# HENDRIX-ZT2/pyaudiorestoration

Hardware: AMD Instinct MI355X
Metric: Msamples/sec resampled (192 kHz varispeed) (higher is better)
Workload: dtype f32 near taps, far taps (|n| >= 3) as float16 hi + lo x 2^-12 filter banks on v_mfma_f32_16x16x32_f16 with f32 accumulation / f64 positions

## Files before the change

pyaudiorestoration_amd/csrc/sinc2.hip:

```cpp
#define PAR_WANT_BANK2 1
#include "par_common.h"
#include "pos_plan.h"
#include "sinc_taps_gen.h"
#include "sinc_common.h"
#define PAR_COLD_FN __forceinline__
#include "sinc_block.h"
#ifndef PAR_COLD_FN_GIVEN
#error "sinc_block.h was included before PAR_COLD_FN was defined: the cold functions would stay out of line"
#endif
#include <algorithm>
#include <atomic>
#include <limits.h>
#include <type_traits>

constexpr int kMaxTilesPerWave = 23;
#ifndef PAR_S2_EXP
#define PAR_S2_EXP 0
#endif

namespace par {

typedef _Float16 half8v __attribute__((ext_vector_type(8)));
typedef _Float16 half2v __attribute__((ext_vector_type(2)));
typedef float float4v __attribute__((ext_vector_type(4)));
// ... 32 lines not shown
  int64_t n_big;
  int64_t n_full;
  int64_t n_tiles;
  int n_edge;
  int64_t out_stride;
  FusedArgs fa;
  const float4* tab;
  TapModes tmd;
};
constexpr int kEdgeWaveOut = 128;
constexpr int kEdgeWavesPerTile = kSincTileOutputs / kEdgeWaveOut;
constexpr int kTileEdge = 0x100;

__device__ __forceinline__ float sinpi_poly(float z) {
  float p = -0.00737043094f;
  p = fmaf(p, z, 0.0821458866f);
  p = fmaf(p, z, -0.599264529f);
  p = fmaf(p, z, 2.55016404f);
  p = fmaf(p, z, -5.16771278f);
  return fmaf(p, z, 3.14159265f);
}

__device__ __forceinline__ _Float16 hi16(float x) { return (_Float16)(fabsf(x) < 6.103515625e-05f ? 0.0f : x); }
#define S2_HI(x) hi16(x)

__device__ __forceinline__ unsigned pack_h2(float a, float b) {
  const half2v h = {(_Float16)a, (_Float16)b};
  return __builtin_bit_cast(unsigned, h);
}
__device__ __forceinline__ float h_lo(unsigned w) { return (float)__builtin_bit_cast(half2v, w)[0]; }
__device__ __forceinline__ float h_hi(unsigned w) { return (float)__builtin_bit_cast(half2v, w)[1]; }


__device__ __forceinline__ void dma_dword(const float* gptr, const void* lds) {
  const unsigned la = (unsigned)(uintptr_t)(const __attribute__((address_space(3))) void*)lds;
  asm volatile("s_mov_b32 m0, %1\n\tglobal_load_lds_dword %0, off" ::"v"(gptr), "s"(__builtin_amdgcn_readfirstlane(la)) : "memory", "m0");
}
__device__ __forceinline__ void dma_dwordx4(const void* gptr, const void* lds) {
  const unsigned la = (unsigned)(uintptr_t)(const __attribute__((address_space(3))) void*)lds;
  asm volatile("s_mov_b32 m0, %1\n\tglobal_load_lds_dwordx4 %0, off" ::"v"(gptr), "s"(__builtin_amdgcn_readfirstlane(la)) : "memory", "m0");
}

__device__ __forceinline__ void dma_chunk128(const float* base, unsigned lane_bytes, const void* lds) {
  const unsigned la = (unsigned)(uintptr_t)(const __attribute__((address_space(3))) void*)lds;
  const unsigned long long b = (unsigned long long)(uintptr_t)base;
  const unsigned long long bs = ((unsigned long long)(unsigned)__builtin_amdgcn_readfirstlane((int)(b >> 32)) << 32) |
                                (unsigned)__builtin_amdgcn_readfirstlane((int)(unsigned)b);
  asm volatile("s_mov_b32 m0, %2\n\tglobal_load_lds_dword %0, %1\n\tglobal_load_lds_dword %0, %1 offset:256"
               ::"v"(lane_bytes), "s"(bs), "s"(__builtin_amdgcn_readfirstlane(la)) : "memory", "m0");
}

__device__ __forceinline__ void dma_chunk256(const float* base, unsigned lane_bytes, const void* lds) {
  const unsigned la = (unsigned)(uintptr_t)(const __attribute__((address_space(3))) void*)lds;
  const unsigned long long b = (unsigned long long)(uintptr_t)base;
  const unsigned long long bs = ((unsigned long long)(unsigned)__builtin_amdgcn_readfirstlane((int)(b >> 32)) << 32) |
                                (unsigned)__builtin_amdgcn_readfirstlane((int)(unsigned)b);
  asm volatile("s_mov_b32 m0, %2\n\tglobal_load_lds_dword %0, %1\n\tglobal_load_lds_dword %0, %1 offset:256\n\t"
               "global_load_lds_dword %0, %1 offset:512\n\tglobal_load_lds_dword %0, %1 offset:768"
               ::"v"(lane_bytes), "s"(bs), "s"(__builtin_amdgcn_readfirstlane(la)) : "memory", "m0");
}

__device__ __forceinline__ void wave_lds_fence() {
  __builtin_amdgcn_fence(__ATOMIC_RELEASE, "wavefront");
  __builtin_amdgcn_wave_barrier();
  __builtin_amdgcn_fence(__ATOMIC_ACQUIRE, "wavefront");
}

__device__ __forceinline__ int clamp64(int n) { return n < 0 ? 0 : (n > 64 ? 64 : n); }
__device__ __forceinline__ unsigned long long prefix(int n) { return n >= 64 ? ~0ull : ((1ull << n) - 1ull); }

struct S2Row {
  int c;
  float s, ep;
  bool bad;
};
template <bool SECOND = true>
__device__ __forceinline__ S2Row s2_place_row(const uint4 ra, const uint4 rb, const int u, const int cbase, const float uf,
                                              const float u2f, const float tw1, const float tw0, const float tolf) {
  const unsigned m = ra.x;
  const bool second = SECOND && (unsigned)u > (m & 31u);
  const float F = __uint_as_float(second ? rb.y : ra.y), e1 = __uint_as_float(second ? rb.z : ra.z),
              e2 = __uint_as_float(second ? rb.w : ra.w);
  const int irel = (int)(second ? rb.x : ra.x) >> 16;
  const bool last = (unsigned)u == ((m >> kRecLastShift) & 63u);
  const float frac = fmaf(u2f, e2, fmaf(uf, e1, F));
  const float e = fmaf(e2, last ? tw0 : tw1, e1);
  const float ri = rintf(frac);
// ... 170 lines not shown
    const float G = 3.14159265f * g, w = G * sr, w2m = w * w, G32 = 32.0f * G;
    float re, im;
    if constexpr (MODE == 3) {
      re = m6 * (1.98412698e-4f * kMs);
      im = 0.0f;
    } else {
      re = m5 * (1.38888889e-3f * kMs);
      im = m5 * (w * -(1.19047619e-3f * kMs));
    }
#define S3_MOM_STEP(Mi, A0, A1, B0)                                   \
    {                                                                 \
      const float al_ = (A1) != 0.0f ? fmaf(w2m, -((A1) * kMs), (A0) * kMs) : (A0) * kMs, be_ = w * -((B0) * kMs);       \
      const float nre_ = fmaf(-G32, im, (Mi) * al_), nim_ = fmaf(G32, re, (Mi) * be_); \
      re = nre_;                                                      \
      im = nim_;                                                      \
    }
    if constexpr (MODE == 3) S3_MOM_STEP(m5, 1.38888889e-3f, 0.0f, 1.19047619e-3f)
    S3_MOM_STEP(m4, 8.33333333e-3f, 0.0f, 6.94444444e-3f)
    S3_MOM_STEP(m3, 4.16666667e-2f, 0.0f, 3.33333333e-2f)
    S3_MOM_STEP(M0[2], 1.66666667e-1f, 5.0e-2f, 1.25e-1f)
    S3_MOM_STEP(M0[1], 0.5f, 0.125f, 3.33333333e-1f)
    S3_MOM_STEP(M0[0], 1.0f, 1.66666667e-1f, 0.5f)
#undef S3_MOM_STEP
    const float S = sr * spq, C = __builtin_amdgcn_cosf(0.5f * sr);
    return fmaf(-g, fmaf(C, re, -(S * im)), unity);
    }
  }
}
template <int MODE, int NCH = 1, class LDS>
__device__ __forceinline__ float s3_out_row(const LDS& L, const int ci, const float sr, const float epr, const int wsK, const int ch = 0) {
  return s3_out_math<MODE>(s3_out_load<MODE, NCH>(L, ci, wsK, ch), sr, epr);
}

template <class LDS>
__device__ __forceinline__ float2 s3_convert_load(const LDS& L, const int chunk, const int l) {
  const int ix = (chunk * kPass + 2 * l) & (kRingF - 1);
  return *reinterpret_cast<const float2*>(&L.ring[ix]);
}
template <class LDS>
__device__ __forceinline__ bool s3_convert_math(LDS& L, const int chunk, const int l, const float2 xx) {
  const int wi = chunk * kPass + 2 * l;
  const int ix = wi & (kRingF - 1), ih = wi & (kRingH - 1);
  const float x0 = xx.x, x1 = xx.y;
  const float am = fmaxf(fabsf(x0), fabsf(x1));
  const bool ok = !(__ballot(!(fabsf(x0) < kImgMax) || !(fabsf(x1) < kImgMax)) != 0ull ||
                    (__ballot(am >= kQuiet) == 0ull && __ballot(am > 0.0f) != 0ull));
  if ((chunk & 7) == 0 && l < 2) *reinterpret_cast<float2*>(&L.ring_tail[ix]) = xx;
  if ((chunk & 7) == 7 && l == kWave - 1) *reinterpret_cast<float2*>(&L.ring_head[2]) = xx;
  const float s0 = x0 * kImgScale, s1 = x1 * kImgScale;
  const half2v h = {S2_HI(s0), S2_HI(s1)};
  const half2v lo = {(_Float16)((s0 - (float)h[0]) * 4096.0f), (_Float16)((s1 - (float)h[1]) * 4096.0f)};
  *reinterpret_cast<half2v*>(&L.img[0][ih]) = h;
  *reinterpret_cast<half2v*>(&L.img[1][ih]) = lo;
  return ok;
}
template <class LDS>
__device__ __forceinline__ bool s3_convert(LDS& L, const int chunk, const int l) {
  return s3_convert_math(L, chunk, l, s3_convert_load(L, chunk, l));
}

template <class LDS>
__device__ __forceinline__ bool s3_convert_ch(LDS& L, const int chunk, const int l, const int ch, const bool mirrors) {
  const int wi = chunk * kPass + 2 * l;
  const int ix = wi & (kRingF - 1), ih = wi & (kRingH - 1);
  const float4v xx = *reinterpret_cast<const float4v*>(&L.ring[2 * ix]);
  const float x0 = ch ? xx[1] : xx[0], x1 = ch ? xx[3] : xx[2];
  const float am = fmaxf(fabsf(x0), fabsf(x1));
  const bool ok = !(__ballot(!(fabsf(x0) < kImgMax) || !(fabsf(x1) < kImgMax)) != 0ull ||
                    (__ballot(am >= kQuiet) == 0ull && __ballot(am > 0.0f) != 0ull));
  if (mirrors) {
    if ((chunk & 7) == 0 && l < 2) *reinterpret_cast<float4v*>(&L.ring_tail[2 * ix]) = xx;
    if ((chunk & 7) == 7 && l == kWave - 1) *reinterpret_cast<float4v*>(&L.ring_head[4]) = xx;
  }
  const float s0 = x0 * kImgScale, s1 = x1 * kImgScale;
  const half2v h = {S2_HI(s0), S2_HI(s1)};
  const half2v lo = {(_Float16)((s0 - (float)h[0]) * 4096.0f), (_Float16)((s1 - (float)h[1]) * 4096.0f)};
  *reinterpret_cast<half2v*>(&L.img[2 * ch][ih]) = h;
  *reinterpret_cast<half2v*>(&L.img[2 * ch + 1][ih]) = lo;
  return ok;
}

constexpr float kEpMaxMom = 0.0125f / (1.0f - 0.0125f);
constexpr float kEpMom5 = 0.0105f / (1.0f - 0.0105f), kEpMom5Lo = 0.95f * kEpMom5;
#ifndef PAR_S3_SHARE_OUT
#define PAR_S3_SHARE_OUT 1
#endif
#ifndef PAR_S3_PIN_MONO
#define PAR_S3_PIN_MONO 0
#endif
template <int NCH, int KIND>
__device__ __forceinline__ void sinc_pipe_body(const S2Args& a, const int bx, S3Lds<NCH, KIND != 1>& L) {
  static_assert(NCH == 1 || NCH == 2, "mono, or an interleaved stereo file");
  static_assert(KIND == 0 || KIND == 3 || NCH == 1, "the stereo form takes every stream");
  static_assert(KIND != 3 || NCH == 2, "one channel of FRAMES");
  constexpr bool kPick = KIND == 3;
  constexpr bool kTwo = NCH == 2 && !kPick;
  constexpr bool kMom = KIND != 1;
  constexpr bool kEarly = NCH == 1 && KIND == 2;
  const int l = threadIdx.x & (kWave - 1);
  if (bx < a.n_edge) {
    if constexpr (KIND == 1) return;
    else {
    const int e = bx / kEdgeWavesPerTile, w = bx % kEdgeWavesPerTile;
    const int64_t T = e == 0 ? 0 : a.n_full - 3 + e;
    const int64_t jw = T * kSincTileOutputs + (int64_t)w * kEdgeWaveOut;
    const int nrem = (int)(a.len_out - jw < (int64_t)kEdgeWaveOut ? (a.len_out - jw > 0 ? a.len_out - jw : 0) : kEdgeWaveOut);
    float* const piece = reinterpret_cast<float*>(&L);
    static_assert(sizeof(L) >= fused_capw(2 * NCH, NCH) * NCH * sizeof(float), "the wave's span fits the stream's LDS");
    if constexpr (kPick) {
      static_assert(sizeof(L) >= fused_capw(2, 1) * sizeof(float), "the wave's span fits the stream's LDS");
      if (nrem > 0)
        fused_wave<1, 32, 2, false>(a.len_out, a.sig, nullptr, 2, a.len_in, 32, a.tab, a.tmd, a.out, nullptr, a.out_stride, a.fa, piece, l,
// ... 27 lines not shown
    if (a.n_edge > 0 && (Ta + l == 0 || Ta + l >= a.n_full - 2)) hd_fl |= 1 | kTileEdge;
    hd_dA = (int)d;
    if constexpr (KIND == 1 || KIND == 2) {
      const bool any_slow = __ballot(l < my_tiles && Ta + l < Tb && (h.flags & kTileMaySlow) != 0) != 0ull;
      if (any_slow != (KIND == 2)) return;
    }
  }
  half8v fr[kBank2Frags];
  {
    const uint4* src = reinterpret_cast<const uint4*>(kBank2Frags32) + l;
#pragma unroll
    for (int f = 0; f < kBank2Frags; ++f) fr[f] = __builtin_bit_cast(half8v, src[f * kWave]);
  }
  half8v fmr[kBank3Frags];
  if constexpr (kMom) {
    const uint4* src = reinterpret_cast<const uint4*>(kBank3Frags32) + l;
#pragma unroll
    for (int f = 0; f < kBank3Frags; ++f) fmr[f] = __builtin_bit_cast(half8v, src[f * kWave]);
  }
  {
    uint4* z = reinterpret_cast<uint4*>(&L.img[0][0]);
    const uint4 zero = {0u, 0u, 0u, 0u};
#pragma unroll
    for (int i = 0; i < (int)(sizeof(L.img) / 16 / kWave); ++i) z[i * kWave + l] = zero;
  }
  const float tolf = (float)((fabs((double)A0) + 2.0e7) * 1.2e-16 + 2.0e-10) + 2.0e-7f;
  const int nJ = (int)(Jb - Ja);
  float* const outW = a.out + (kPick ? a.out_stride : (int64_t)NCH) * Ja;
  const uint4* const recW = reinterpret_cast<const uint4*>(a.rec) + (Ja >> kRecShift);
  const uint4* const rec2W = reinterpret_cast<const uint4*>(a.rec2) + (Ja >> kRecShift);
  const int blk_max = (int)(((a.len_out + kRec - 1) >> kRecShift) - (Ja >> kRecShift)) - 1;

  int j0 = 0;
  int wbase = 0, conv_next = 0, conv_lo = 0, dma_next = 0, dma_bad = INT_MAX, mode = 0, pk = 0;
  int regime = 1;
  int rbA = 0, rbB = 0, rbC = 0;

  const uint4* const rec_lane = (l < 8 ? recW : rec2W) + (l & 7);
  auto fetch_records = [&](int buf, int blk0) {
    if (l < 16) dma_dwordx4(rec_lane + (blk0 < 0 ? 0 : blk0), &L.recs[buf][0]);
  };
  int dma_klo = 0, dma_khi = -1;
  const float* ring_src = a.sig;
  auto ring_restart = [&]() {
    const long long o = A0 + wbase;
    ring_src = a.sig + NCH * o;
    const long long klo = o >= 0 ? 0 : (-o + kPass - 1) / kPass, khi = ((long long)a.len_in - (kPick ? 1 : 0) - o) / kPass - 1;
    dma_klo = (int)(klo > 0x3fffffff ? 0x3fffffff : klo);
    dma_khi = (int)(khi > 0x3fffffff ? 0x3fffffff : (khi < -1 ? -1 : khi));
  };
  const unsigned lane_bytes = 4u * (unsigned)l;
  auto chunk_dma = [&](int k) {
    const bool inside = k >= dma_klo && k <= dma_khi;
    if (!inside) dma_bad = k < dma_bad ? k : dma_bad;
    const float* src = inside ? ring_src + (long long)(kPass * NCH) * k : a.sig;
    if constexpr (NCH == 2) dma_chunk256(src, lane_bytes, &L.ring[(k & 7) * (kPass * 2)]);
    else dma_chunk128(src, lane_bytes, &L.ring[(k & 7) * kPass]);
  };
  auto push_tile = [&](int64_t T) {
    if (l == 0) {
      const int slot = atomicAdd(a.redo_count, 1);
      a.redo_list[slot] = (int)T;
    }
  };
  if (stream_id == 0 && a.n_full < a.n_tiles && a.n_edge == 0) push_tile(a.n_full);

  struct Placed {
    S2Row R[2];
    int nt[2];
    int fl0, fl1, tend;
    int epm;
  };
  int tc_T = -1, tc_dA0 = 0, tc_dA1 = 0, tc_fl0 = 0, tc_fl1 = 0;
  struct PlaceRecs {
    uint4 ra0, rb0, ra1, rb1;
  };
  auto place_load = [&](int j, int buf, int rb) {
    const int t5 = (j & (kRec - 1)) + l;
    const int bi = ((j >> kRecShift) - rb + (t5 >> kRecShift)) & 7;
    const uint4* rp = &L.recs[buf][0];
    return PlaceRecs{rp[bi], rp[8 + bi], rp[(bi + 2) & 7], rp[8 + ((bi + 2) & 7)]};
  };
  auto place_impl = [&](int j, int buf, int rb, auto early, const PlaceRecs& RR) {
    Placed P;
    const int T = j >> 10;
    P.tend = (T + 1) << 10;
    if (T != tc_T) {
      tc_T = T;
      tc_dA0 = __builtin_amdgcn_readlane(hd_dA, T);
      tc_dA1 = __builtin_amdgcn_readlane(hd_dA, T + 1);
      tc_fl0 = __builtin_amdgcn_readlane(hd_fl, T);
      tc_fl1 = __builtin_amdgcn_readlane(hd_fl, T + 1);
    }
    const int dA0 = tc_dA0, dA1 = tc_dA1;
    P.fl0 = tc_fl0;
    P.fl1 = tc_fl1;
    const int t5 = (j & (kRec - 1)) + l;
    const int u = t5 & (kRec - 1);
    uint4 ra0, rb0, ra1, rb1;
    if constexpr (decltype(early)::value) {
      ra0 = RR.ra0, rb0 = RR.rb0, ra1 = RR.ra1, rb1 = RR.rb1;
    } else {
      const int bi = ((j >> kRecShift) - rb + (t5 >> kRecShift)) & 7;
      const uint4* rp = &L.recs[buf][0];
      ra0 = rp[bi], rb0 = rp[8 + bi], ra1 = rp[(bi + 2) & 7], rb1 = rp[8 + ((bi + 2) & 7)];
    }
    const int uc = u - kRec / 2;
    const float uf = (float)uc, u2f = uf * uf, tw1 = fmaf(2.0f, uf, 1.0f), tw0 = tw1 - 2.0f;
    P.nt[0] = clamp64(P.tend - j);
    P.nt[1] = clamp64(P.tend - j - 64);
    if (__ballot((unsigned)u > (ra0.x & 31u) || (unsigned)u > (ra1.x & 31u)) == 0ull) {
      P.R[0] = s2_place_row<false>(ra0, rb0, u, (l < P.nt[0] ? dA0 : dA1) + uc, uf, u2f, tw1, tw0, tolf);
      P.R[1] = s2_place_row<false>(ra1, rb1, u, (l < P.nt[1] ? dA0 : dA1) + uc, uf, u2f, tw1, tw0, tolf);
    } else {
      P.R[0] = s2_place_row(ra0, rb0, u, (l < P.nt[0] ? dA0 : dA1) + uc, uf, u2f, tw1, tw0, tolf);
      P.R[1] = s2_place_row(ra1, rb1, u, (l < P.nt[1] ? dA0 : dA1) + uc, uf, u2f, tw1, tw0, tolf);
    }
    P.epm = max(__float_as_int(P.R[0].ep), __float_as_int(P.R[1].ep));
    return P;
  };
  auto place = [&](int j, int buf, int rb) { return place_impl(j, buf, rb, std::false_type{}, PlaceRecs{}); };

  S3Pass P;
  P.nok[0] = P.nok[1] = 0;
  P.j = P.ws = 0;
  P.c[0] = P.c[1] = 0;
  P.s[0] = P.s[1] = P.ep[0] = P.ep[1] = 0.0f;

  auto out_pass = [&](auto mode_tag, const S3Pass& Q, float (&res)[2], const int ch = 0) {
    constexpr int MODE = decltype(mode_tag)::value;
    const int wsK = Q.ws - wbase;
#pragma unroll
    for (int r = 0; r < 2; ++r) {
      int ci = Q.c[r] - Q.ws;
      ci = ci < 0 ? 0 : (ci > kPass - 1 ? kPass - 1 : ci);
      float sr = Q.s[r], epr = Q.ep[r];
#if !PAR_S3_SHARE_OUT
      if (NCH == 2 && ch == 1) asm volatile("" : "+v"(sr), "+v"(epr));
#endif
      res[r] = s3_out_row<MODE, NCH>(L, ci, sr, epr, wsK, ch);
    }
  };
  auto store_pass = [&](const S3Pass& Q, const float (&res)[2]) {
#pragma unroll
    for (int r = 0; r < 2; ++r)
      if (l < Q.nok[r] && !(PAR_S2_EXP & 4)) {
        if constexpr (kPick) outW[(int64_t)((unsigned)Q.j + 64u * r + (unsigned)l) * a.out_stride] = res[r];
        else outW[(unsigned)Q.j + 64u * r + (unsigned)l] = res[r];
      }
  };
  auto store_pass2 = [&](const S3Pass& Q, const float (&res0)[2], const float (&res1)[2]) {
#pragma unroll
    for (int r = 0; r < 2; ++r)
      if (l < Q.nok[r] && !(PAR_S2_EXP & 4))
        reinterpret_cast<float2*>(outW)[(unsigned)Q.j + 64u * r + (unsigned)l] = make_float2(res0[r], res1[r]);
  };
  auto convert_chunk = [&](int chunk) -> bool {
    if constexpr (kPick) {
      return s3_convert_ch(L, chunk, l, 0, true);
    } else if constexpr (NCH == 2) {
      const bool ok0 = s3_convert_ch(L, chunk, l, 0, true);
      const bool ok1 = s3_convert_ch(L, chunk, l, 1, false);
      return ok0 && ok1;
    } else {
      return s3_convert(L, chunk, l);
    }
  };

#if PAR_S2_EXP & 128
#define S3_COUNT(k) do { if (l == 0) atomicAdd(a.redo_count + (k), 1); } while (0)
#else
#define S3_COUNT(k) do { } while (0)
#endif
  auto start_run = [&]() -> bool {
    for (;;) {
      if (j0 >= nJ) return false;
      S3_COUNT(1);
      __builtin_amdgcn_s_waitcnt(0x0F70);
      wave_lds_fence();
      const int buf = pk & 3;
      fetch_records(buf, j0 >> kRecShift);
      __builtin_amdgcn_s_waitcnt(0x0F70);
      wave_lds_fence();
      const Placed Q = place(j0, buf, j0 >> kRecShift);
      const int tend = Q.tend;
      int nv[2] = {clamp64(nJ - j0), clamp64(nJ - j0 - 64)};
      const unsigned long long b0 = __ballot(Q.R[0].bad || !(Q.R[0].ep <= kEpMaxMom)) & prefix(nv[0]),
                               b1 = __ballot(Q.R[1].bad || !(Q.R[1].ep <= kEpMaxMom)) & prefix(nv[1]);
      const unsigned long long bad_here = (b0 & prefix(Q.nt[0])) | (b1 & prefix(Q.nt[1]));
      const bool bad_next = ((b0 & ~prefix(Q.nt[0])) | (b1 & ~prefix(Q.nt[1])) | (unsigned long long)((Q.fl1 & 1) && tend < nJ)) != 0ull;
      if (bad_next) {
        nv[0] = nv[0] < Q.nt[0] ? nv[0] : Q.nt[0];
        nv[1] = nv[1] < Q.nt[1] ? nv[1] : Q.nt[1];
      }
      bool skip = (Q.fl0 & 1) || bad_here != 0ull;
      const unsigned long long gen = (__ballot(1.0f + Q.R[0].ep != 1.0f) & prefix(nv[0])) | (__ballot(1.0f + Q.R[1].ep != 1.0f) & prefix(nv[1]));
      const int ws = __builtin_amdgcn_readfirstlane(Q.R[0].c) & ~7;
      S3Pass N;
#pragma unroll
      for (int r = 0; r < 2; ++r) {
        N.c[r] = Q.R[r].c;
        N.s[r] = Q.R[r].s;
        N.ep[r] = Q.R[r].ep;
        const unsigned long long in = __ballot(Q.R[r].c - ws < kPass);
        N.nok[r] = __popcll(in & prefix(nv[r]));
      }
      N.j = j0;
      N.ws = ws;
      const unsigned long long steep = (__ballot(Q.R[0].ep > kEpMom5) & prefix(nv[0])) | (__ballot(Q.R[1].ep > kEpMom5) & prefix(nv[1]));
      const int want = gen == 0ull ? 1 : (steep == 0ull ? 2 : 3);
      if (!kMom && want != 1) skip = true;
      if (!skip) {
        bool rebuild = mode != 1;
        const int lo_need = ws - 39 - wbase;
        if (mode == 0 || lo_need < kPass * (dma_next - 8) + kPass || lo_need < 0 || lo_need > kPass * dma_next || ws - wbase > (1 << 20)) {
          __builtin_amdgcn_s_waitcnt(0x0F70);
          wbase = ws - 39;
          dma_next = 0;
          dma_bad = INT_MAX;
          rebuild = true;
          ring_restart();
        }
        const int wsK = ws - wbase;
        regime = want;
        if (rebuild) {
          mode = 1;
          conv_lo = conv_next = (wsK - 39) >> 7;
        }
        const int conv_target = want == 1 ? (wsK + 300 + 127) >> 7 : (wsK + 465) >> 7;
        const int need_lo = (wsK - 39) >> 7;
        if (conv_next < need_lo) conv_lo = conv_next = need_lo;
        int conv_end = conv_target > conv_next ? conv_target : conv_next;
        if (need_lo < conv_lo || need_lo < conv_end - 4) {
          conv_lo = conv_next = need_lo;
          conv_end = conv_target > need_lo ? conv_target : need_lo;
        }
        while (dma_next < conv_end + 2) chunk_dma(dma_next++);
        const int jn = j0 + N.nok[0] + N.nok[1];
        rbA = jn >> kRecShift;
        rbB = (jn + 120) >> kRecShift;
        fetch_records((pk + 1) & 3, rbA);
        fetch_records((pk + 2) & 3, rbB);
        __builtin_amdgcn_s_waitcnt(0x0F70);
        wave_lds_fence();
        if (!skip) {
#pragma unroll 1
          while (conv_next < conv_end) {
            if (conv_next >= dma_bad) {
              skip = true;
              break;
            }
            const bool ok = convert_chunk(conv_next);
            if (!ok) {
              skip = true;
              break;
            }
            ++conv_next;
          }
        }
        if (!skip && conv_next + 1 >= dma_bad) skip = true;
      }
      if (skip) {
        if (!(Q.fl0 & kTileEdge)) push_tile(Ta + (j0 >> 10));
        j0 = tend;
        mode = 0;
        continue;
      }
      wave_lds_fence();
      const int offs = ws - wbase - 31;
      if (kMom && regime == 3) bank_image3m<kMom, true>(L, fr, fmr, offs, l);
      else if (kMom && regime == 2) bank_image3m<kMom, false>(L, fr, fmr, offs, l);
      else bank_image3m<false>(L, fr, fmr, offs, l);
      wave_lds_fence();
      j0 += N.nok[0] + N.nok[1];
      ++pk;
      rbC = (j0 + 240) >> kRecShift;
      const bool full = N.nok[1] >= 1 && N.nok[0] + N.nok[1] >= 120;
      if (full) {
        P = N;
        return true;
      }
      float res[2];
      if (kMom && regime == 3) out_pass(std::integral_constant<int, kMom ? 3 : 1>{}, N, res);
      else if (kMom && regime == 2) out_pass(std::integral_constant<int, kMom ? 2 : 1>{}, N, res);
      else out_pass(std::integral_constant<int, 1>{}, N, res);
      if constexpr (kTwo) {
        float res1[2];
        wave_lds_fence();
        if (regime == 3) bank_image3m<true, true>(L, fr, fmr, offs, l, 1);
        else if (regime == 2) bank_image3m<true, false>(L, fr, fmr, offs, l, 1);
        else bank_image3m<false>(L, fr, fmr, offs, l, 1);
        wave_lds_fence();
        if (regime == 3) out_pass(std::integral_constant<int, 3>{}, N, res1, 1);
        else if (regime == 2) out_pass(std::integral_constant<int, 2>{}, N, res1, 1);
        else out_pass(std::integral_constant<int, 1>{}, N, res1, 1);
        store_pass2(N, res, res1);
      } else {
        store_pass(N, res);
      }
    }
  };

#if PAR_S2_EXP & 64
  unsigned long long s3t_[4] = {0, 0, 0, 0}, s3last_ = __builtin_readcyclecounter();
  const unsigned long long s3start_ = s3last_;
#endif
  auto hot = [&](auto mode_tag) {
    constexpr int MODE = decltype(mode_tag)::value;
    j0 = __builtin_amdgcn_readfirstlane(j0);
    wbase = __builtin_amdgcn_readfirstlane(wbase);
    conv_next = __builtin_amdgcn_readfirstlane(conv_next);
    dma_next = __builtin_amdgcn_readfirstlane(dma_next);
    dma_bad = __builtin_amdgcn_readfirstlane(dma_bad);
    pk = __builtin_amdgcn_readfirstlane(pk);
    rbA = __builtin_amdgcn_readfirstlane(rbA);
    rbB = __builtin_amdgcn_readfirstlane(rbB);
    rbC = __builtin_amdgcn_readfirstlane(rbC);
    for (;;) {
#if PAR_S2_EXP & 64
      const unsigned long long tA_ = __builtin_readcyclecounter();
#endif
      if constexpr (NCH == 2) asm volatile("s_waitcnt vmcnt(7)" ::: "memory");
      else asm volatile("s_waitcnt vmcnt(5)" ::: "memory");
#if PAR_S2_EXP & 64
      const unsigned long long tB_ = __builtin_readcyclecounter();
      s3t_[0] += tB_ - tA_;
      s3t_[1] += tA_ - s3last_;
      s3last_ = tB_;
      s3t_[2] += 1;
#endif
      wave_lds_fence();
      S3Pass N;
      bool ok;
      int wsK;
      auto place_next = [&](auto early, const PlaceRecs& RR) {
      const Placed Q = place_impl(j0, pk & 3, rbA, early, RR);
      const unsigned long long bad = __ballot(Q.R[0].bad || Q.R[1].bad || Q.epm > __float_as_int(kEpMaxMom));
      const unsigned long long gen = __ballot(Q.epm > 0x33800000);
      bool tier = true;
      if constexpr (MODE == 2) tier = __ballot(Q.epm > __float_as_int(kEpMom5)) == 0ull;
      if constexpr (MODE == 3) tier = __ballot(Q.epm > __float_as_int(kEpMom5Lo)) != 0ull;
      const int ws = __builtin_amdgcn_readfirstlane(Q.R[0].c) & ~7;
#pragma unroll
      for (int r = 0; r < 2; ++r) {
        N.c[r] = Q.R[r].c;
        N.s[r] = Q.R[r].s;
        N.ep[r] = Q.R[r].ep;
        N.nok[r] = __popcll(__ballot(Q.R[r].c - ws < kPass));
      }
      N.j = j0;
      N.ws = ws;
      wsK = ws - wbase;
      const int d = kPass * conv_next - wsK;
      ok = (((Q.fl0 | Q.fl1) & 1) == 0) & (bad == 0ull) & (j0 + kPass <= nJ) & (N.nok[0] + N.nok[1] >= 120) &
           (MODE == 1 ? gen == 0ull : gen != 0ull) & tier & ((unsigned)(d - 161) <= 312u) & (conv_next + 1 < dma_bad) &
           ((unsigned)((j0 >> kRecShift) - rbA) <= 1u);
      };
      float res[2];
      bool cok;
      if constexpr (kEarly) {
        const PlaceRecs RR = place_load(j0, pk & 3, rbA);
        const float2 cxx = s3_convert_load(L, conv_next, l);
        S3Gather G[2];
        const int wsP = P.ws - wbase;
#pragma unroll
        for (int r = 0; r < 2; ++r) {
          int ci = P.c[r] - P.ws;
          ci = ci < 0 ? 0 : (ci > kPass - 1 ? kPass - 1 : ci);
          G[r] = s3_out_load<MODE, NCH>(L, ci, wsP);
        }
        __builtin_amdgcn_sched_barrier(0);
        place_next(std::true_type{}, RR);
        const S3Frags X = bank_load(L, wsK - 31, l);
        __builtin_amdgcn_sched_barrier(0);
        if constexpr (MODE == 2) {
          res[0] = s3_out_math<MODE>(G[0], P.s[0], P.ep[0]);
          asm volatile("" : "+v"(res[0]));
          asm volatile("" ::"v"(G[0].Mh[3]));
          __builtin_amdgcn_sched_barrier(0);
          res[1] = s3_out_math<MODE>(G[1], P.s[1], P.ep[1]);
          bank_math<true, false>(L, fr, fmr, X, l);
          asm volatile("" : "+v"(res[1]));
          asm volatile("" ::"v"(G[1].Mh[3]));
#pragma unroll
          for (int i = 0; i < 28; ++i) {
            __builtin_amdgcn_sched_group_barrier(0x008, 1, 0);
            __builtin_amdgcn_sched_group_barrier(0x002, 2, 0);
          }
        } else {
#pragma unroll
          for (int r = 0; r < 2; ++r) res[r] = s3_out_math<MODE>(G[r], P.s[r], P.ep[r]);
          asm volatile("" : "+v"(res[0]), "+v"(res[1]));
          __builtin_amdgcn_sched_barrier(0);
          bank_math<MODE != 1, MODE == 3>(L, fr, fmr, X, l);
        }
        int oki = __builtin_amdgcn_readfirstlane((int)ok);
        asm volatile("" : "+s"(oki));
        ok = oki != 0;
        cok = s3_convert_math(L, conv_next, l, cxx);
        fetch_records((pk + 2) & 3, rbC);
        chunk_dma(dma_next);
        store_pass(P, res);
      } else {
      if constexpr (!kTwo) place_next(std::false_type{}, PlaceRecs{});
      out_pass(mode_tag, P, res);
      if constexpr (kTwo) {
        float res1[2];
        asm volatile("" : "+v"(res[0]), "+v"(res[1]));
        bank_image3m<MODE != 1, MODE == 3>(L, fr, fmr, P.ws - wbase - 31, l, 1);
        out_pass(mode_tag, P, res1, 1);
        asm volatile("" : "+v"(res1[0]), "+v"(res1[1]));
        place_next(std::false_type{}, PlaceRecs{});
        const int offs = wsK - 31;
        bank_image3m<MODE != 1, MODE == 3>(L, fr, fmr, offs, l, 0);
        const bool c0 = s3_convert_ch(L, conv_next, l, 0, true);
        const bool c1 = s3_convert_ch(L, conv_next - 1, l, 1, false);
        cok = c0 && c1;
        fetch_records((pk + 2) & 3, rbC);
        chunk_dma(dma_next);
        store_pass2(P, res, res1);
      } else {
        const int offs = wsK - 31;
#if PAR_S3_PIN_MONO
        asm volatile("" : "+v"(res[0]), "+v"(res[1]));
#endif
        bank_image3m<MODE != 1, MODE == 3>(L, fr, fmr, offs, l);
        cok = convert_chunk(conv_next);
        fetch_records((pk + 2) & 3, rbC);
        chunk_dma(dma_next);
        store_pass(P, res);
      }
      }
      wave_lds_fence();
      ++conv_next;
      ++dma_next;
      if (!cok) mode = 0;
      S3_COUNT(2);
#if PAR_S2_EXP & 128
      if (!(ok && cok)) {
        if (((Q.fl0 | Q.fl1) & 1) != 0 || bad != 0ull) S3_COUNT(3);
        else if (!(j0 + kPass <= nJ)) S3_COUNT(4);
        else if (!(N.nok[1] >= 1 && N.nok[0] + N.nok[1] >= 120)) S3_COUNT(5);
        else if (!(MODE == 1 ? gen == 0ull : gen != 0ull)) S3_COUNT(6);
        else if (!(d >= 161 && d <= 473)) S3_COUNT(7);
        else if (!(conv_next < dma_bad)) S3_COUNT(9);
        else if (!((unsigned)((j0 >> kRecShift) - rbA) <= 1u)) S3_COUNT(11);
        else if (!cok) S3_COUNT(10);
        else S3_COUNT(8);
      }
#endif
      if (!(ok && cok)) {
        if constexpr (kTwo)
          if (mode != 0 && !s3_convert_ch(L, conv_next - 1, l, 1, false)) mode = 0;
        return;
      }
      P = N;
      j0 += N.nok[0] + N.nok[1];
      ++pk;
      rbA = rbB;
      rbB = rbC;
      rbC = (j0 + 240) >> kRecShift;
    }
  };

  while (start_run()) {
    if (kMom && regime == 3) hot(std::integral_constant<int, kMom ? 3 : 1>{});
    else if (kMom && regime == 2) hot(std::integral_constant<int, kMom ? 2 : 1>{});
    else hot(std::integral_constant<int, 1>{});
  }
  __builtin_amdgcn_s_waitcnt(0x0F70);
#if PAR_S2_EXP & 64
  if (l == 0) {
    unsigned long long* o = g_s2_phase + (size_t)stream_id * 16;
    o[0] = s3t_[0];
    o[1] = s3t_[1];
    o[2] = s3t_[2];
    o[3] = __builtin_readcyclecounter() - s3start_;
    o[6] = s3t_[2];
  }
#endif
}

template <int NCH, int KIND>
__global__ __launch_bounds__(kWave, KIND == 1 ? 3 : 2) void k_sinc_pipe(const S2Args a) {
  __shared__ S3Lds<NCH, KIND != 1> L;
  sinc_pipe_body<NCH, KIND>(a, (int)blockIdx.x, L);
}

constexpr int kBatchFiles = kFusedBatchMax;
struct S2Batch {
  int n;
  int first[kBatchFiles + 1];
  S2Args f[kBatchFiles];
};
static_assert(sizeof(S2Batch) <= 3584, "kernel arguments fit the 4 KB segment");
// ... 105 lines not shown
```

Before: 175,000.

## Strength-reduce hot-loop bookkeeping and fold exit checks into one integer margin

```diff
diff --git a/pyaudiorestoration_amd/csrc/sinc2.hip b/pyaudiorestoration_amd/csrc/sinc2.hip
--- a/pyaudiorestoration_amd/csrc/sinc2.hip
+++ b/pyaudiorestoration_amd/csrc/sinc2.hip
@@ -88,27 +88,24 @@
 __device__ __forceinline__ float h_hi(unsigned w) { return (float)__builtin_bit_cast(half2v, w)[1]; }
 
 
-__device__ __forceinline__ void dma_dword(const float* gptr, const void* lds) {
-  const unsigned la = (unsigned)(uintptr_t)(const __attribute__((address_space(3))) void*)lds;
+__device__ __forceinline__ unsigned lds_addr(const void* lds) {
+  return (unsigned)(uintptr_t)(const __attribute__((address_space(3))) void*)lds;
+}
+__device__ __forceinline__ void dma_dword(const float* gptr, const unsigned la) {
   asm volatile("s_mov_b32 m0, %1\n\tglobal_load_lds_dword %0, off" ::"v"(gptr), "s"(__builtin_amdgcn_readfirstlane(la)) : "memory", "m0");
 }
-__device__ __forceinline__ void dma_dwordx4(const void* gptr, const void* lds) {
-  const unsigned la = (unsigned)(uintptr_t)(const __attribute__((address_space(3))) void*)lds;
+__device__ __forceinline__ void dma_dwordx4(const void* gptr, const unsigned la) {
   asm volatile("s_mov_b32 m0, %1\n\tglobal_load_lds_dwordx4 %0, off" ::"v"(gptr), "s"(__builtin_amdgcn_readfirstlane(la)) : "memory", "m0");
 }
 
-__device__ __forceinline__ void dma_chunk128(const float* base, unsigned lane_bytes, const void* lds) {
-  const unsigned la = (unsigned)(uintptr_t)(const __attribute__((address_space(3))) void*)lds;
-  const unsigned long long b = (unsigned long long)(uintptr_t)base;
+__device__ __forceinline__ void dma_chunk128(const unsigned long long b, unsigned lane_bytes, const unsigned la) {
   const unsigned long long bs = ((unsigned long long)(unsigned)__builtin_amdgcn_readfirstlane((int)(b >> 32)) << 32) |
                                 (unsigned)__builtin_amdgcn_readfirstlane((int)(unsigned)b);
   asm volatile("s_mov_b32 m0, %2\n\tglobal_load_lds_dword %0, %1\n\tglobal_load_lds_dword %0, %1 offset:256"
                ::"v"(lane_bytes), "s"(bs), "s"(__builtin_amdgcn_readfirstlane(la)) : "memory", "m0");
 }
 
-__device__ __forceinline__ void dma_chunk256(const float* base, unsigned lane_bytes, const void* lds) {
-  const unsigned la = (unsigned)(uintptr_t)(const __attribute__((address_space(3))) void*)lds;
-  const unsigned long long b = (unsigned long long)(uintptr_t)base;
+__device__ __forceinline__ void dma_chunk256(const unsigned long long b, unsigned lane_bytes, const unsigned la) {
   const unsigned long long bs = ((unsigned long long)(unsigned)__builtin_amdgcn_readfirstlane((int)(b >> 32)) << 32) |
                                 (unsigned)__builtin_amdgcn_readfirstlane((int)(unsigned)b);
   asm volatile("s_mov_b32 m0, %2\n\tglobal_load_lds_dword %0, %1\n\tglobal_load_lds_dword %0, %1 offset:256\n\t"
@@ -345,52 +342,62 @@
   return s3_out_math<MODE>(s3_out_load<MODE, NCH>(L, ci, wsK, ch), sr, epr);
 }
 
+__device__ __forceinline__ unsigned long long s3_convert_verdict(const float x0, const float x1) {
+  const float am = fmaxf(fabsf(x0), fabsf(x1));
+  const unsigned long long big = __ballot(!(fabsf(x0) < kImgMax) || !(fabsf(x1) < kImgMax));
+  const unsigned long long loud = __ballot(am >= kQuiet), some = __ballot(am > 0.0f);
+  return big | (loud == 0ull ? some : 0ull);
+}
+template <int NCH, class LDS, class V>
+__device__ __forceinline__ void s3_ring_mirrors(LDS& L, const int w0, const int l, const int ix, const V xx) {
+  const int slot = w0 & (7 * kPass);
+  if (slot == 0) {
+    __builtin_amdgcn_wave_barrier();
+    if (l < 2) *reinterpret_cast<V*>(&L.ring_tail[NCH * ix]) = xx;
+  }
+  if (slot == 7 * kPass) {
+    __builtin_amdgcn_wave_barrier();
+    if (l == kWave - 1) *reinterpret_cast<V*>(&L.ring_head[2 * NCH]) = xx;
+  }
+}
 template <class LDS>
-__device__ __forceinline__ float2 s3_convert_load(const LDS& L, const int chunk, const int l) {
-  const int ix = (chunk * kPass + 2 * l) & (kRingF - 1);
+__device__ __forceinline__ float2 s3_convert_load(const LDS& L, const int w0, const int l) {
+  const int ix = (w0 + 2 * l) & (kRingF - 1);
   return *reinterpret_cast<const float2*>(&L.ring[ix]);
 }
 template <class LDS>
-__device__ __forceinline__ bool s3_convert_math(LDS& L, const int chunk, const int l, const float2 xx) {
-  const int wi = chunk * kPass + 2 * l;
+__device__ __forceinline__ unsigned long long s3_convert_math(LDS& L, const int w0, const int l, const float2 xx) {
+  const int wi = w0 + 2 * l;
   const int ix = wi & (kRingF - 1), ih = wi & (kRingH - 1);
   const float x0 = xx.x, x1 = xx.y;
-  const float am = fmaxf(fabsf(x0), fabsf(x1));
-  const bool ok = !(__ballot(!(fabsf(x0) < kImgMax) || !(fabsf(x1) < kImgMax)) != 0ull ||
-                    (__ballot(am >= kQuiet) == 0ull && __ballot(am > 0.0f) != 0ull));
-  if ((chunk & 7) == 0 && l < 2) *reinterpret_cast<float2*>(&L.ring_tail[ix]) = xx;
-  if ((chunk & 7) == 7 && l == kWave - 1) *reinterpret_cast<float2*>(&L.ring_head[2]) = xx;
+  const unsigned long long trouble = s3_convert_verdict(x0, x1);
+  s3_ring_mirrors<1>(L, w0, l, ix, xx);
   const float s0 = x0 * kImgScale, s1 = x1 * kImgScale;
   const half2v h = {S2_HI(s0), S2_HI(s1)};
   const half2v lo = {(_Float16)((s0 - (float)h[0]) * 4096.0f), (_Float16)((s1 - (float)h[1]) * 4096.0f)};
   *reinterpret_cast<half2v*>(&L.img[0][ih]) = h;
   *reinterpret_cast<half2v*>(&L.img[1][ih]) = lo;
-  return ok;
+  return trouble;
 }
 template <class LDS>
-__device__ __forceinline__ bool s3_convert(LDS& L, const int chunk, const int l) {
-  return s3_convert_math(L, chunk, l, s3_convert_load(L, chunk, l));
+__device__ __forceinline__ unsigned long long s3_convert(LDS& L, const int w0, const int l) {
+  return s3_convert_math(L, w0, l, s3_convert_load(L, w0, l));
 }
 
 template <class LDS>
-__device__ __forceinline__ bool s3_convert_ch(LDS& L, const int chunk, const int l, const int ch, const bool mirrors) {
-  const int wi = chunk * kPass + 2 * l;
+__device__ __forceinline__ unsigned long long s3_convert_ch(LDS& L, const int w0, const int l, const int ch, const bool mirrors) {
+  const int wi = w0 + 2 * l;
   const int ix = wi & (kRingF - 1), ih = wi & (kRingH - 1);
   const float4v xx = *reinterpret_cast<const float4v*>(&L.ring[2 * ix]);
   const float x0 = ch ? xx[1] : xx[0], x1 = ch ? xx[3] : xx[2];
-  const float am = fmaxf(fabsf(x0), fabsf(x1));
-  const bool ok = !(__ballot(!(fabsf(x0) < kImgMax) || !(fabsf(x1) < kImgMax)) != 0ull ||
-                    (__ballot(am >= kQuiet) == 0ull && __ballot(am > 0.0f) != 0ull));
-  if (mirrors) {
-    if ((chunk & 7) == 0 && l < 2) *reinterpret_cast<float4v*>(&L.ring_tail[2 * ix]) = xx;
-    if ((chunk & 7) == 7 && l == kWave - 1) *reinterpret_cast<float4v*>(&L.ring_head[4]) = xx;
-  }
+  const unsigned long long trouble = s3_convert_verdict(x0, x1);
+  if (mirrors) s3_ring_mirrors<2>(L, w0, l, ix, xx);
   const float s0 = x0 * kImgScale, s1 = x1 * kImgScale;
   const half2v h = {S2_HI(s0), S2_HI(s1)};
   const half2v lo = {(_Float16)((s0 - (float)h[0]) * 4096.0f), (_Float16)((s1 - (float)h[1]) * 4096.0f)};
   *reinterpret_cast<half2v*>(&L.img[2 * ch][ih]) = h;
   *reinterpret_cast<half2v*>(&L.img[2 * ch + 1][ih]) = lo;
-  return ok;
+  return trouble;
 }
 
 constexpr float kEpMaxMom = 0.0125f / (1.0f - 0.0125f);
@@ -484,30 +491,36 @@
   const int blk_max = (int)(((a.len_out + kRec - 1) >> kRecShift) - (Ja >> kRecShift)) - 1;
 
   int j0 = 0;
-  int wbase = 0, conv_next = 0, conv_lo = 0, dma_next = 0, dma_bad = INT_MAX, mode = 0, pk = 0;
+  constexpr int kDmaBadMax = 1 << 22;
+  int wbase = 0, conv_next = 0, conv_lo = 0, dma_next = 0, dma_bad = 0, mode = 0, pk = 0;
   int regime = 1;
   int rbA = 0, rbB = 0, rbC = 0;
 
   const uint4* const rec_lane = (l < 8 ? recW : rec2W) + (l & 7);
-  auto fetch_records = [&](int buf, int blk0) {
-    if (l < 16) dma_dwordx4(rec_lane + (blk0 < 0 ? 0 : blk0), &L.recs[buf][0]);
-  };
-  int dma_klo = 0, dma_khi = -1;
-  const float* ring_src = a.sig;
+  using LdsT = S3Lds<NCH, KIND != 1>;
+  const unsigned lds_base = lds_addr(&L);
+  const unsigned lds_recs = lds_base + (unsigned)offsetof(LdsT, recs), lds_ring = lds_base + (unsigned)offsetof(LdsT, ring);
+  constexpr unsigned kRecBufBytes = 16 * sizeof(uint4);
+  constexpr unsigned kChunkBytes = kPass * NCH * sizeof(float);
+  auto fetch_records_at = [&](unsigned rbytes, int blk0) {
+    if (l < 16) dma_dwordx4(rec_lane + (blk0 < 0 ? 0 : blk0), lds_recs + rbytes);
+  };
+  auto fetch_records = [&](int buf, int blk0) { fetch_records_at(kRecBufBytes * (unsigned)buf, blk0); };
+  unsigned long long ring_src = (unsigned long long)(uintptr_t)a.sig;
   auto ring_restart = [&]() {
     const long long o = A0 + wbase;
-    ring_src = a.sig + NCH * o;
-    const long long klo = o >= 0 ? 0 : (-o + kPass - 1) / kPass, khi = ((long long)a.len_in - (kPick ? 1 : 0) - o) / kPass - 1;
-    dma_klo = (int)(klo > 0x3fffffff ? 0x3fffffff : klo);
-    dma_khi = (int)(khi > 0x3fffffff ? 0x3fffffff : (khi < -1 ? -1 : khi));
+    ring_src = (unsigned long long)(uintptr_t)a.sig + (unsigned long long)((long long)(NCH * sizeof(float)) * o);
+    const long long khi = ((long long)a.len_in - (kPick ? 1 : 0) - o) / kPass - 1;
+    dma_bad = o < 0 || khi < 0 ? 0 : (int)(khi + 1 > kDmaBadMax ? kDmaBadMax : khi + 1);
   };
   const unsigned lane_bytes = 4u * (unsigned)l;
+  auto chunk_dma_at = [&](bool inside, unsigned long long src, unsigned slot_bytes) {
+    const unsigned long long s = inside ? src : (unsigned long long)(uintptr_t)a.sig;
+    if constexpr (NCH == 2) dma_chunk256(s, lane_bytes, lds_ring + slot_bytes);
+    else dma_chunk128(s, lane_bytes, lds_ring + slot_bytes);
+  };
   auto chunk_dma = [&](int k) {
-    const bool inside = k >= dma_klo && k <= dma_khi;
-    if (!inside) dma_bad = k < dma_bad ? k : dma_bad;
-    const float* src = inside ? ring_src + (long long)(kPass * NCH) * k : a.sig;
-    if constexpr (NCH == 2) dma_chunk256(src, lane_bytes, &L.ring[(k & 7) * (kPass * 2)]);
-    else dma_chunk128(src, lane_bytes, &L.ring[(k & 7) * kPass]);
+    chunk_dma_at(k < dma_bad, ring_src + (unsigned long long)((long long)kChunkBytes * k), (unsigned)(k & 7) * kChunkBytes);
   };
   auto push_tile = [&](int64_t T) {
     if (l == 0) {
@@ -523,27 +536,28 @@
     int fl0, fl1, tend;
     int epm;
   };
-  int tc_T = -1, tc_dA0 = 0, tc_dA1 = 0, tc_fl0 = 0, tc_fl1 = 0;
+  int tc_tend = 0, tc_dA0 = 0, tc_dA1 = 0, tc_fl0 = 0, tc_fl1 = 0, tc_flm = 0;
   struct PlaceRecs {
     uint4 ra0, rb0, ra1, rb1;
   };
-  auto place_load = [&](int j, int buf, int rb) {
+  auto place_load = [&](int j, unsigned rbytes, int jb) {
     const int t5 = (j & (kRec - 1)) + l;
-    const int bi = ((j >> kRecShift) - rb + (t5 >> kRecShift)) & 7;
-    const uint4* rp = &L.recs[buf][0];
+    const int bi = (jb + (t5 >> kRecShift)) & 7;
+    const uint4* rp = &L.recs[0][0] + (rbytes >> 4);
     return PlaceRecs{rp[bi], rp[8 + bi], rp[(bi + 2) & 7], rp[8 + ((bi + 2) & 7)]};
   };
-  auto place_impl = [&](int j, int buf, int rb, auto early, const PlaceRecs& RR) {
+  auto place_impl = [&](int j, unsigned rbytes, int jb, auto early, const PlaceRecs& RR) {
     Placed P;
-    const int T = j >> 10;
-    P.tend = (T + 1) << 10;
-    if (T != tc_T) {
-      tc_T = T;
+    if (j >= tc_tend) {
+      const int T = j >> 10;
+      tc_tend = (T + 1) << 10;
       tc_dA0 = __builtin_amdgcn_readlane(hd_dA, T);
       tc_dA1 = __builtin_amdgcn_readlane(hd_dA, T + 1);
       tc_fl0 = __builtin_amdgcn_readlane(hd_fl, T);
       tc_fl1 = __builtin_amdgcn_readlane(hd_fl, T + 1);
-    }
+      tc_flm = -((tc_fl0 | tc_fl1) & 1);
+    }
+    P.tend = tc_tend;
     const int dA0 = tc_dA0, dA1 = tc_dA1;
     P.fl0 = tc_fl0;
     P.fl1 = tc_fl1;
@@ -553,14 +567,14 @@
     if constexpr (decltype(early)::value) {
       ra0 = RR.ra0, rb0 = RR.rb0, ra1 = RR.ra1, rb1 = RR.rb1;
     } else {
-      const int bi = ((j >> kRecShift) - rb + (t5 >> kRecShift)) & 7;
-      const uint4* rp = &L.recs[buf][0];
+      const int bi = (jb + (t5 >> kRecShift)) & 7;
+      const uint4* rp = &L.recs[0][0] + (rbytes >> 4);
       ra0 = rp[bi], rb0 = rp[8 + bi], ra1 = rp[(bi + 2) & 7], rb1 = rp[8 + ((bi + 2) & 7)];
     }
     const int uc = u - kRec / 2;
     const float uf = (float)uc, u2f = uf * uf, tw1 = fmaf(2.0f, uf, 1.0f), tw0 = tw1 - 2.0f;
-    P.nt[0] = clamp64(P.tend - j);
-    P.nt[1] = clamp64(P.tend - j - 64);
+    P.nt[0] = P.tend - j;
+    P.nt[1] = P.tend - j - 64;
     if (__ballot((unsigned)u > (ra0.x & 31u) || (unsigned)u > (ra1.x & 31u)) == 0ull) {
       P.R[0] = s2_place_row<false>(ra0, rb0, u, (l < P.nt[0] ? dA0 : dA1) + uc, uf, u2f, tw1, tw0, tolf);
       P.R[1] = s2_place_row<false>(ra1, rb1, u, (l < P.nt[1] ? dA0 : dA1) + uc, uf, u2f, tw1, tw0, tolf);
@@ -571,7 +585,9 @@
     P.epm = max(__float_as_int(P.R[0].ep), __float_as_int(P.R[1].ep));
     return P;
   };
-  auto place = [&](int j, int buf, int rb) { return place_impl(j, buf, rb, std::false_type{}, PlaceRecs{}); };
+  auto place = [&](int j, int buf, int rb) {
+    return place_impl(j, kRecBufBytes * (unsigned)buf, (j >> kRecShift) - rb, std::false_type{}, PlaceRecs{});
+  };
 
   S3Pass P;
   P.nok[0] = P.nok[1] = 0;
@@ -607,15 +623,15 @@
       if (l < Q.nok[r] && !(PAR_S2_EXP & 4))
         reinterpret_cast<float2*>(outW)[(unsigned)Q.j + 64u * r + (unsigned)l] = make_float2(res0[r], res1[r]);
   };
-  auto convert_chunk = [&](int chunk) -> bool {
+  auto convert_chunk = [&](int w0) -> unsigned long long {
     if constexpr (kPick) {
-      return s3_convert_ch(L, chunk, l, 0, true);
+      return s3_convert_ch(L, w0, l, 0, true);
     } else if constexpr (NCH == 2) {
-      const bool ok0 = s3_convert_ch(L, chunk, l, 0, true);
-      const bool ok1 = s3_convert_ch(L, chunk, l, 1, false);
-      return ok0 && ok1;
+      const unsigned long long t0 = s3_convert_ch(L, w0, l, 0, true);
+      const unsigned long long t1 = s3_convert_ch(L, w0, l, 1, false);
+      return t0 | t1;
     } else {
-      return s3_convert(L, chunk, l);
+      return s3_convert(L, w0, l);
     }
   };
 
@@ -639,11 +655,12 @@
       int nv[2] = {clamp64(nJ - j0), clamp64(nJ - j0 - 64)};
       const unsigned long long b0 = __ballot(Q.R[0].bad || !(Q.R[0].ep <= kEpMaxMom)) & prefix(nv[0]),
                                b1 = __ballot(Q.R[1].bad || !(Q.R[1].ep <= kEpMaxMom)) & prefix(nv[1]);
-      const unsigned long long bad_here = (b0 & prefix(Q.nt[0])) | (b1 & prefix(Q.nt[1]));
-      const bool bad_next = ((b0 & ~prefix(Q.nt[0])) | (b1 & ~prefix(Q.nt[1])) | (unsigned long long)((Q.fl1 & 1) && tend < nJ)) != 0ull;
+      const int nt0 = clamp64(Q.nt[0]), nt1 = clamp64(Q.nt[1]);
+      const unsigned long long bad_here = (b0 & prefix(nt0)) | (b1 & prefix(nt1));
+      const bool bad_next = ((b0 & ~prefix(nt0)) | (b1 & ~prefix(nt1)) | (unsigned long long)((Q.fl1 & 1) && tend < nJ)) != 0ull;
       if (bad_next) {
-        nv[0] = nv[0] < Q.nt[0] ? nv[0] : Q.nt[0];
-        nv[1] = nv[1] < Q.nt[1] ? nv[1] : Q.nt[1];
+        nv[0] = nv[0] < nt0 ? nv[0] : nt0;
+        nv[1] = nv[1] < nt1 ? nv[1] : nt1;
       }
       bool skip = (Q.fl0 & 1) || bad_here != 0ull;
       const unsigned long long gen = (__ballot(1.0f + Q.R[0].ep != 1.0f) & prefix(nv[0])) | (__ballot(1.0f + Q.R[1].ep != 1.0f) & prefix(nv[1]));
@@ -669,7 +686,6 @@
           __builtin_amdgcn_s_waitcnt(0x0F70);
           wbase = ws - 39;
           dma_next = 0;
-          dma_bad = INT_MAX;
           rebuild = true;
           ring_restart();
         }
@@ -702,7 +718,7 @@
               skip = true;
               break;
             }
-            const bool ok = convert_chunk(conv_next);
+            const bool ok = convert_chunk(kPass * conv_next) == 0ull;
             if (!ok) {
               skip = true;
               break;
@@ -761,13 +777,24 @@
     constexpr int MODE = decltype(mode_tag)::value;
     j0 = __builtin_amdgcn_readfirstlane(j0);
     wbase = __builtin_amdgcn_readfirstlane(wbase);
-    conv_next = __builtin_amdgcn_readfirstlane(conv_next);
-    dma_next = __builtin_amdgcn_readfirstlane(dma_next);
-    dma_bad = __builtin_amdgcn_readfirstlane(dma_bad);
-    pk = __builtin_amdgcn_readfirstlane(pk);
     rbA = __builtin_amdgcn_readfirstlane(rbA);
     rbB = __builtin_amdgcn_readfirstlane(rbB);
     rbC = __builtin_amdgcn_readfirstlane(rbC);
+    tc_tend = __builtin_amdgcn_readfirstlane(tc_tend);
+    tc_flm = __builtin_amdgcn_readfirstlane(tc_flm);
+    const int cn0 = __builtin_amdgcn_readfirstlane(conv_next), pk0 = __builtin_amdgcn_readfirstlane(pk);
+    const int dn0 = __builtin_amdgcn_readfirstlane(dma_next), dbad = __builtin_amdgcn_readfirstlane(dma_bad);
+    int w0 = kPass * cn0;
+    unsigned rbytes = kRecBufBytes * (unsigned)(pk0 & 3);
+    unsigned dslot = kChunkBytes * (unsigned)(dn0 & 7);
+    unsigned long long dsrc = ring_src + (unsigned long long)((long long)kChunkBytes * dn0);
+    dsrc = ((unsigned long long)(unsigned)__builtin_amdgcn_readfirstlane((int)(dsrc >> 32)) << 32) |
+           (unsigned)__builtin_amdgcn_readfirstlane((int)(unsigned)dsrc);
+    const int nJm = nJ - kPass;
+    const int cn_lim = kPass * (dbad - 2);
+    const int dn_lim = kPass * (dbad - (dn0 - cn0));
+    unsigned long long cok = 0ull;
+    int m = 0, adv = 0;
     for (;;) {
 #if PAR_S2_EXP & 64
       const unsigned long long tA_ = __builtin_readcyclecounter();
@@ -783,15 +810,16 @@
 #endif
       wave_lds_fence();
       S3Pass N;
-      bool ok;
       int wsK;
+      const int jb = (j0 >> kRecShift) - rbA;
       auto place_next = [&](auto early, const PlaceRecs& RR) {
-      const Placed Q = place_impl(j0, pk & 3, rbA, early, RR);
-      const unsigned long long bad = __ballot(Q.R[0].bad || Q.R[1].bad || Q.epm > __float_as_int(kEpMaxMom));
-      const unsigned long long gen = __ballot(Q.epm > 0x33800000);
-      bool tier = true;
-      if constexpr (MODE == 2) tier = __ballot(Q.epm > __float_as_int(kEpMom5)) == 0ull;
-      if constexpr (MODE == 3) tier = __ballot(Q.epm > __float_as_int(kEpMom5Lo)) != 0ull;
+      const Placed Q = place_impl(j0, rbytes, jb, early, RR);
+      constexpr int kEpGen = 0x33800000;
+      const int ep_hi = MODE == 1 ? kEpGen : (MODE == 2 ? __float_as_int(kEpMom5) : __float_as_int(kEpMaxMom));
+      const int n_none = __popcll(__ballot(Q.R[0].bad || Q.R[1].bad || Q.epm > ep_hi));
+      int n_some = 1;
+      if constexpr (MODE == 2) n_some = __popcll(__ballot(Q.epm > kEpGen));
+      if constexpr (MODE == 3) n_some = __popcll(__ballot(Q.epm > __float_as_int(kEpMom5Lo)));
       const int ws = __builtin_amdgcn_readfirstlane(Q.R[0].c) & ~7;
 #pragma unroll
       for (int r = 0; r < 2; ++r) {
@@ -803,16 +831,19 @@
       N.j = j0;
       N.ws = ws;
       wsK = ws - wbase;
-      const int d = kPass * conv_next - wsK;
-      ok = (((Q.fl0 | Q.fl1) & 1) == 0) & (bad == 0ull) & (j0 + kPass <= nJ) & (N.nok[0] + N.nok[1] >= 120) &
-           (MODE == 1 ? gen == 0ull : gen != 0ull) & tier & ((unsigned)(d - 161) <= 312u) & (conv_next + 1 < dma_bad) &
-           ((unsigned)((j0 >> kRecShift) - rbA) <= 1u);
+      const int d = w0 - wsK;
+      adv = N.nok[0] + N.nok[1];
+      m = min(tc_flm, nJm - j0);
+      m = min(m, adv - 120 - 16 * n_none);
+      m = min(m, min(d - 161, 473 - d));
+      m = min(m, cn_lim - w0);
+      m = min(m, min(jb, 1 - jb));
+      if constexpr (MODE != 1) m = min(m, n_some - 1);
       };
       float res[2];
-      bool cok;
       if constexpr (kEarly) {
-        const PlaceRecs RR = place_load(j0, pk & 3, rbA);
-        const float2 cxx = s3_convert_load(L, conv_next, l);
+        const PlaceRecs RR = place_load(j0, rbytes, jb);
+        const float2 cxx = s3_convert_load(L, w0, l);
         S3Gather G[2];
         const int wsP = P.ws - wbase;
 #pragma unroll
@@ -846,12 +877,11 @@
           __builtin_amdgcn_sched_barrier(0);
           bank_math<MODE != 1, MODE == 3>(L, fr, fmr, X, l);
         }
-        int oki = __builtin_amdgcn_readfirstlane((int)ok);
-        asm volatile("" : "+s"(oki));
-        ok = oki != 0;
-        cok = s3_convert_math(L, conv_next, l, cxx);
-        fetch_records((pk + 2) & 3, rbC);
-        chunk_dma(dma_next);
+        m = __builtin_amdgcn_readfirstlane(m);
+        asm volatile("" : "+s"(m));
+        cok = s3_convert_math(L, w0, l, cxx);
+        fetch_records_at(rbytes ^ (2 * kRecBufBytes), rbC);
+        chunk_dma_at(w0 < dn_lim, dsrc, dslot);
         store_pass(P, res);
       } else {
       if constexpr (!kTwo) place_next(std::false_type{}, PlaceRecs{});
@@ -865,11 +895,11 @@
         place_next(std::false_type{}, PlaceRecs{});
         const int offs = wsK - 31;
         bank_image3m<MODE != 1, MODE == 3>(L, fr, fmr, offs, l, 0);
-        const bool c0 = s3_convert_ch(L, conv_next, l, 0, true);
-        const bool c1 = s3_convert_ch(L, conv_next - 1, l, 1, false);
-        cok = c0 && c1;
-        fetch_records((pk + 2) & 3, rbC);
-        chunk_dma(dma_next);
+        const unsigned long long c0 = s3_convert_ch(L, w0, l, 0, true);
+        const unsigned long long c1 = s3_convert_ch(L, w0 - kPass, l, 1, false);
+        cok = c0 | c1;
+        fetch_records_at(rbytes ^ (2 * kRecBufBytes), rbC);
+        chunk_dma_at(w0 < dn_lim, dsrc, dslot);
         store_pass2(P, res, res1);
       } else {
         const int offs = wsK - 31;
@@ -877,42 +907,31 @@
         asm volatile("" : "+v"(res[0]), "+v"(res[1]));
 #endif
         bank_image3m<MODE != 1, MODE == 3>(L, fr, fmr, offs, l);
-        cok = convert_chunk(conv_next);
-        fetch_records((pk + 2) & 3, rbC);
-        chunk_dma(dma_next);
+        cok = convert_chunk(w0);
+        fetch_records_at(rbytes ^ (2 * kRecBufBytes), rbC);
+        chunk_dma_at(w0 < dn_lim, dsrc, dslot);
         store_pass(P, res);
       }
       }
       wave_lds_fence();
-      ++conv_next;
-      ++dma_next;
-      if (!cok) mode = 0;
+      w0 += kPass;
+      dsrc += kChunkBytes;
+      dslot = (dslot + kChunkBytes) & (8 * kChunkBytes - 1);
       S3_COUNT(2);
-#if PAR_S2_EXP & 128
-      if (!(ok && cok)) {
-        if (((Q.fl0 | Q.fl1) & 1) != 0 || bad != 0ull) S3_COUNT(3);
-        else if (!(j0 + kPass <= nJ)) S3_COUNT(4);
-        else if (!(N.nok[1] >= 1 && N.nok[0] + N.nok[1] >= 120)) S3_COUNT(5);
-        else if (!(MODE == 1 ? gen == 0ull : gen != 0ull)) S3_COUNT(6);
-        else if (!(d >= 161 && d <= 473)) S3_COUNT(7);
-        else if (!(conv_next < dma_bad)) S3_COUNT(9);
-        else if (!((unsigned)((j0 >> kRecShift) - rbA) <= 1u)) S3_COUNT(11);
-        else if (!cok) S3_COUNT(10);
-        else S3_COUNT(8);
-      }
-#endif
-      if (!(ok && cok)) {
-        if constexpr (kTwo)
-          if (mode != 0 && !s3_convert_ch(L, conv_next - 1, l, 1, false)) mode = 0;
-        return;
-      }
+      if (min(m, -(int)__popcll(cok)) < 0) break;
       P = N;
-      j0 += N.nok[0] + N.nok[1];
-      ++pk;
+      j0 += adv;
+      rbytes = (rbytes + kRecBufBytes) & (3 * kRecBufBytes);
       rbA = rbB;
       rbB = rbC;
       rbC = (j0 + 240) >> kRecShift;
     }
+    conv_next = w0 >> 7;
+    dma_next = dn0 + (conv_next - cn0);
+    pk = pk0 + (conv_next - cn0) - 1;
+    if (cok != 0ull) mode = 0;
+    if constexpr (kTwo)
+      if (mode != 0 && s3_convert_ch(L, w0 - kPass, l, 1, false) != 0ull) mode = 0;
   };
 
   while (start_run()) {
```

New measurement: 181,200, median of 6. 3.6% higher.
